# leonardsiegert/PULPo

Measured on AMD Instinct MI355X. Metric: volume-pairs/sec fwd+bwd, 160^3 fp32, higher is better.
Workload: dtype f32

## Files before the change

pulpo_amd/csrc/losses.hip:

```cpp
#include "common.h"

namespace {

inline int eblocks(long items, int cap = 4096) { return (int)std::max<long>(1, std::min<long>((items + 255) / 256, cap)); }

__device__ __forceinline__ float block_sum_256(float v, float* sh) {
    v = pulpo::wave_sum(v);
    if ((threadIdx.x & 63) == 0) sh[threadIdx.x >> 6] = v;
    __syncthreads();
    float t = 0.f;
    if (threadIdx.x == 0) t = sh[0] + sh[1] + sh[2] + sh[3];
    __syncthreads();
    return t;
}

__device__ __forceinline__ float ncc_cc(const float* s, float nwin) {
    const float uI = s[0] / nwin, uJ = s[1] / nwin;
    const float cross = s[4] - uJ * s[0] - uI * s[1] + uI * uJ * nwin;
    const float Iv = s[2] - 2.f * uI * s[0] + uI * uI * nwin;
    const float Jv = s[3] - 2.f * uJ * s[1] + uJ * uJ * nwin;
    return cross * cross / (Iv * Jv + 1e-8f);
}

__device__ __forceinline__ float mask_weight(const float* __restrict__ wa, const float* __restrict__ wb, long e) {
    return wb != nullptr ? wa[e] * wb[e] : wa[e];
}

template <bool MASKED>
__device__ __forceinline__ void store_block_partials(float local, float msum, float* sh, float* __restrict__ partial) {
    const float t = block_sum_256(local, sh);
    if constexpr (MASKED) {
        const float tm = block_sum_256(msum, sh);
        if (threadIdx.x == 0) {
            partial[2 * blockIdx.x] = t;
            partial[2 * blockIdx.x + 1] = tm;
        }
    } else {
        if (threadIdx.x == 0) partial[blockIdx.x] = t;
    }
}

template <int MODE>
__global__ __launch_bounds__(256) void box_x_kernel(const float* __restrict__ in0, const float* __restrict__ in1, float* __restrict__ out, long N,
                                                      long nrows, int W, int pad, int nch, int segs_per_row) {
    const int lane = threadIdx.x & 63;
    const int span = 64 - 2 * pad;
    const long nwork = nrows * segs_per_row;
    const long wave0 = (blockIdx.x * (long)blockDim.x + threadIdx.x) >> 6;
    const long nwave = ((long)gridDim.x * blockDim.x) >> 6;
    for (long wk = wave0; wk < nwork; wk += nwave) {
        const long row = wk / segs_per_row;
        const int seg = (int)(wk - row * segs_per_row);
        const int x = seg * span - pad + lane;
        const bool inb = x >= 0 && x < W;
        const long idx = row * W + x;
        const bool owner = lane >= pad && lane < 64 - pad && x < W;
        if constexpr (MODE == 0) {
            const float I = inb ? in0[idx] : 0.f, J = inb ? in1[idx] : 0.f;
            float v[5] = {I, J, I * I, J * J, I * J};
            float s[5] = {v[0], v[1], v[2], v[3], v[4]};
            for (int k = 1; k <= pad; ++k) {
#pragma unroll
                for (int c = 0; c < 5; ++c) s[c] += __shfl(v[c], lane - k, 64) + __shfl(v[c], lane + k, 64);
            }
            if (owner) {
#pragma unroll
                for (int c = 0; c < 5; ++c) out[c * N + idx] = s[c];
            }
        } else {
            for (int c = 0; c < nch; ++c) {
                const float v = inb ? in0[c * N + idx] : 0.f;
                float s = v;
                for (int k = 1; k <= pad; ++k) s += __shfl(v, lane - k, 64) + __shfl(v, lane + k, 64);
                if (owner) out[c * N + idx] = s;
            }
        }
    }
}

__global__ __launch_bounds__(256) void box_axis_kernel(const float* __restrict__ in, float* __restrict__ out, long N, int nch, int extent, long stride,
                                                         int pad) {
    for (long e = blockIdx.x * (long)blockDim.x + threadIdx.x; e < N; e += (long)gridDim.x * blockDim.x) {
        const int pos = (int)((e / stride) % extent);
        const int lo = max(-pad, -pos), hi = min(pad, extent - 1 - pos);
        for (int c = 0; c < nch; ++c) {
            const float* s = in + c * N + e;
            float acc = 0.f;
            for (int k = lo; k <= hi; ++k) acc += s[k * stride];
            out[c * N + e] = acc;
        }
    }
}

template <bool MASKED>
__global__ __launch_bounds__(256) void ncc_final_kernel(const float* __restrict__ in, float* __restrict__ S, long N, int extent, long stride, int pad,
                                                          float nwin, const float* __restrict__ wa, const float* __restrict__ wb, float* __restrict__ partial) {
    __shared__ float sh[4];
    float local = 0.f;
    [[maybe_unused]] float msum = 0.f;
    for (long e = blockIdx.x * (long)blockDim.x + threadIdx.x; e < N; e += (long)gridDim.x * blockDim.x) {
        const int pos = (int)((e / stride) % extent);
        const int lo = max(-pad, -pos), hi = min(pad, extent - 1 - pos);
        float s[5];
#pragma unroll
        for (int c = 0; c < 5; ++c) {
            const float* q = in + c * N + e;
            float acc = 0.f;
            for (int k = lo; k <= hi; ++k) acc += q[k * stride];
            s[c] = acc;
            S[c * N + e] = acc;
        }
        if constexpr (MASKED) {
            const float m = mask_weight(wa, wb, e);
            local += m * ncc_cc(s, nwin);
            msum += m;
        } else {
            local += ncc_cc(s, nwin);
        }
    }
    store_block_partials<MASKED>(local, msum, sh, partial);
}

template <int NCH, int PAD, int MODE, bool MASKED>
__global__ __launch_bounds__(256) void box_march_kernel(const float* __restrict__ in, float* __restrict__ out, long N, long nlines, int extent,
                                                          long stride, int seglen, int nseg, float nwin, float* __restrict__ partial,
                                                          const float* __restrict__ I, const float* __restrict__ J, const float* __restrict__ gscale,
                                                          float coef, const float* __restrict__ wa, const float* __restrict__ wb) {
    constexpr int WIN = 2 * PAD + 1;
    __shared__ float sh[4];
    const long nlg = (nlines + 255) / 256;
    const long nitem = nlg * nseg;
    float local = 0.f;
    [[maybe_unused]] float msum = 0.f;
    [[maybe_unused]] const float k0 = MODE == 2 ? coef * (gscale != nullptr ? gscale[0] : 1.f) : 0.f;
    for (long item = blockIdx.x; item < nitem; item += gridDim.x) {
        const long lg = item % nlg;
        const int seg = (int)(item / nlg);
        const long line = lg * 256 + threadIdx.x;
        if (line >= nlines) continue;
        const long outer = line / stride, inner = line - outer * stride;
        const long base = outer * extent * stride + inner;
        const int p0 = seg * seglen, p1 = min(extent, p0 + seglen);
        float ring[NCH][WIN];
#pragma unroll
        for (int j = 0; j < WIN - 1; ++j) {
            const int pos = p0 - PAD + j;
            const bool ok = pos >= 0 && pos < extent;
#pragma unroll
            for (int c = 0; c < NCH; ++c) ring[c][j] = ok ? in[c * N + base + pos * stride] : 0.f;
        }
        for (int t0 = p0; t0 < p1; t0 += WIN) {
#pragma unroll
            for (int u = 0; u < WIN; ++u) {
                const int p = t0 + u;
                if (p < p1) {
                    const int slot = (u + WIN - 1) % WIN;
                    const int pos = p + PAD;
                    const bool ok = pos < extent;
                    float sum[NCH];
#pragma unroll
                    for (int c = 0; c < NCH; ++c) {
                        ring[c][slot] = ok ? in[c * N + base + pos * stride] : 0.f;
                        float acc = 0.f;
#pragma unroll
                        for (int j = 0; j < WIN; ++j) acc += ring[c][(u + j) % WIN];
                        sum[c] = acc;
                    }
                    const long e = base + p * stride;
                    if constexpr (MODE == 0) {
#pragma unroll
                        for (int c = 0; c < NCH; ++c) out[c * N + e] = sum[c];
                    } else if constexpr (MODE == 1) {
#pragma unroll
                        for (int c = 0; c < NCH; ++c) out[c * N + e] = sum[c];
                        if constexpr (MASKED) {
                            const float m = mask_weight(wa, wb, e);
                            local += m * ncc_cc(sum, nwin);
                            msum += m;
                        } else {
                            local += ncc_cc(sum, nwin);
                        }
                    } else {
                        out[e] = k0 * (sum[0] + 2.f * J[e] * sum[1] + I[e] * sum[2]);
                    }
                }
            }
        }
    }
    if constexpr (MODE == 1) store_block_partials<MASKED>(local, msum, sh, partial);
}

static inline void march_segments(long nlines, int extent, int pad, int& seglen, int& nseg) {
    const long nlg = (nlines + 255) / 256;
    const long want = std::max<long>(1, (1024 + nlg - 1) / nlg);
    nseg = (int)std::max<long>(1, std::min<long>(want, extent / std::max(1, 2 * pad)));
    seglen = (extent + nseg - 1) / nseg;
    nseg = (extent + seglen - 1) / seglen;
}

template <int NCH, int MODE, bool MASKED = false>
static int launch_march(int pad, int grid, hipStream_t st, const float* in, float* out, long N, int extent, long stride, float nwin = 0.f,
                        float* partial = nullptr, const float* I = nullptr, const float* J = nullptr, const float* gscale = nullptr, float coef = 0.f,
                        const float* wa = nullptr, const float* wb = nullptr) {
    const long nlines = N / extent;
    int seglen, nseg;
    march_segments(nlines, extent, pad, seglen, nseg);
#define PULPO_MARCH(P) hipLaunchKernelGGL((box_march_kernel<NCH, P, MODE, MASKED>), dim3(grid), dim3(256), 0, st, in, out, N, nlines, extent, stride, seglen, nseg, nwin, partial, I, J, gscale, coef, wa, wb)
    switch (pad) {
        case 1: PULPO_MARCH(1); break;
        case 2: PULPO_MARCH(2); break;
        case 3: PULPO_MARCH(3); break;
        case 4: PULPO_MARCH(4); break;
        case 5: PULPO_MARCH(5); break;
        default: return -1;
    }
#undef PULPO_MARCH
    return pulpo::check_launch("ncc box march");
}

template <bool MASKED>
__global__ __launch_bounds__(256) void ncc_abc_kernel(const float* __restrict__ S, float* __restrict__ A, long N, float nwin,
                                                        const float* __restrict__ wa, const float* __restrict__ wb) {
    for (long e = blockIdx.x * (long)blockDim.x + threadIdx.x; e < N; e += (long)gridDim.x * blockDim.x) {
        const float SI = S[e], SJ = S[N + e], SII = S[2 * N + e], SJJ = S[3 * N + e], SIJ = S[4 * N + e];
        const float cross = SIJ - SI * SJ / nwin;
        const float Iv = SII - SI * SI / nwin;
        const float Jv = SJJ - SJ * SJ / nwin;
        const float Dn = Iv * Jv + 1e-8f;
        const float r = cross / Dn;
        float a = -2.f * r * SI / nwin + 2.f * r * r * Iv * SJ / nwin, b = -r * r * Iv, c = 2.f * r;
        if constexpr (MASKED) {
            const float m = mask_weight(wa, wb, e);
            a = m * a, b = m * b, c = m * c;
        }
        A[e] = a;
        A[N + e] = b;
        A[2 * N + e] = c;
    }
}

__global__ __launch_bounds__(256) void masked_finish_kernel(const float* __restrict__ partial, int nblk, double scale, int root, double count,
                                                              float* __restrict__ out) {
    __shared__ double red[2][256];
    double s = 0.0, m = 0.0;
    for (int r = threadIdx.x; r < nblk; r += 256) {
        s += (double)partial[2 * r];
        m += (double)partial[2 * r + 1];
    }
    red[0][threadIdx.x] = s;
    red[1][threadIdx.x] = m;
    __syncthreads();
    for (int half = 128; half > 0; half >>= 1) {
        if ((int)threadIdx.x < half) {
            red[0][threadIdx.x] += red[0][threadIdx.x + half];
            red[1][threadIdx.x] += red[1][threadIdx.x + half];
        }
        __syncthreads();
    }
    if (threadIdx.x == 0) {
        const double S0 = red[0][0], M = red[1][0];
        const bool live = M > 0.0;
        const double q = live ? scale * S0 / M : 0.0;
        double val = q, dval = live ? scale / M : 0.0;
        if (root) {
            val = q > 0.0 ? sqrt(q) : 0.0;
            dval = q > 0.0 ? dval / (2.0 * val) : 0.0;
        }
        out[0] = (float)val;
        out[1] = (float)dval;
        out[2] = (float)(M / count);
        out[3] = (float)M;
    }
}

__global__ __launch_bounds__(256) void ncc_bwd_final_kernel(const float* __restrict__ in, const float* __restrict__ I, const float* __restrict__ J,
                                                              const float* __restrict__ gscale, float coef, float* __restrict__ gJ, long N, int extent,
                                                              long stride, int pad) {
    const float k0 = coef * (gscale != nullptr ? gscale[0] : 1.f);
    for (long e = blockIdx.x * (long)blockDim.x + threadIdx.x; e < N; e += (long)gridDim.x * blockDim.x) {
        const int pos = (int)((e / stride) % extent);
        const int lo = max(-pad, -pos), hi = min(pad, extent - 1 - pos);
        float s[3];
#pragma unroll
        for (int c = 0; c < 3; ++c) {
            const float* q = in + c * N + e;
            float acc = 0.f;
            for (int k = lo; k <= hi; ++k) acc += q[k * stride];
            s[c] = acc;
        }
        gJ[e] = k0 * (s[0] + 2.f * J[e] * s[1] + I[e] * s[2]);
    }
}

__global__ __launch_bounds__(256) void kl_fwd_kernel(const float* __restrict__ mu, const float* __restrict__ sigma, const float* __restrict__ mu1,
                                                       const float* __restrict__ sigma1, long n, float* __restrict__ partial) {
    __shared__ float sh[4];
    float local = 0.f;
    const float eps = 1e-10f;
    for (long e = blockIdx.x * (long)blockDim.x + threadIdx.x; e < n; e += (long)gridDim.x * blockDim.x) {
        const float s0 = sigma[e] * sigma[e];
        const float s1 = sigma1 != nullptr ? sigma1[e] * sigma1[e] : 1.f;
        const float dm = (mu1 != nullptr ? mu1[e] : 0.f) - mu[e];
        local += (s0 + dm * dm) / (s1 + eps) + logf(s1 + eps) - logf(s0 + eps) - 1.f;
    }
    const float t = block_sum_256(local, sh);
    if (threadIdx.x == 0) partial[blockIdx.x] = t;
}

__global__ __launch_bounds__(256) void kl_bwd_kernel(const float* __restrict__ mu, const float* __restrict__ sigma, const float* __restrict__ mu1,
                                                       const float* __restrict__ sigma1, const float* __restrict__ gscale, float coef,
                                                       float* __restrict__ gmu, float* __restrict__ gsigma, long n) {
    const float k0 = coef * (gscale != nullptr ? gscale[0] : 1.f);
    const float eps = 1e-10f;
    for (long e = blockIdx.x * (long)blockDim.x + threadIdx.x; e < n; e += (long)gridDim.x * blockDim.x) {
        const float s = sigma[e], m = mu[e];
        const float s1 = sigma1 != nullptr ? sigma1[e] * sigma1[e] : 1.f;
        const float m1 = mu1 != nullptr ? mu1[e] : 0.f;
        gmu[e] = k0 * (m - m1) / (s1 + eps);
        gsigma[e] = k0 * (s / (s1 + eps) - s / (s * s + eps));
    }
}

__global__ __launch_bounds__(256) void l2reg_fwd_kernel(const float* __restrict__ df, long nplanes, int D, int H, int W, float* __restrict__ partial) {
    __shared__ float sh[4];
    float local = 0.f;
    const long V = (long)D * H * W, total = nplanes * V;
    for (long e = blockIdx.x * (long)blockDim.x + threadIdx.x; e < total; e += (long)gridDim.x * blockDim.x) {
        const long v = e % V;
        const int x = (int)(v % W), y = (int)((v / W) % H), z = (int)(v / ((long)W * H));
        if (x >= 1 && y >= 1 && (z >= 1 || D == 1)) {
            const float c = df[e];
            const float a = D == 1 ? 0.f : c - df[e - (long)H * W], b = c - df[e - W], d = c - df[e - 1];
            local += a * a + b * b + d * d;
        }
    }
    const float t = block_sum_256(local, sh);
    if (threadIdx.x == 0) partial[blockIdx.x] = t;
}

__global__ __launch_bounds__(256) void l2reg_fwd_vec_kernel(const float* __restrict__ df, long nplanes, int D, int H, int W, float* __restrict__ partial) {
    __shared__ float sh[4];
    float local = 0.f;
    const int W4 = W >> 2;
    const long items = nplanes * D * H * W4;
    for (long it = blockIdx.x * (long)blockDim.x + threadIdx.x; it < items; it += (long)gridDim.x * blockDim.x) {
        const int x4 = (int)(it % W4);
        const long row = it / W4;
        const int y = (int)(row % H);
        const int z = (int)((row / H) % D);
        if (y >= 1 && (z >= 1 || D == 1)) {
            const long e = row * W + 4 * x4;
            const float4 c = *reinterpret_cast<const float4*>(df + e);
            const float4 u = *reinterpret_cast<const float4*>(df + e - W);
            float4 bk = c;
            if (D != 1) bk = *reinterpret_cast<const float4*>(df + e - (long)H * W);
            const float cc[4] = {c.x, c.y, c.z, c.w}, uu[4] = {u.x, u.y, u.z, u.w}, bb[4] = {bk.x, bk.y, bk.z, bk.w};
            float left = x4 > 0 ? df[e - 1] : 0.f;
#pragma unroll
            for (int k = 0; k < 4; ++k) {
                if (4 * x4 + k >= 1) {
                    const float a = cc[k] - bb[k], b = cc[k] - uu[k], d = cc[k] - left;
                    local += a * a + b * b + d * d;
                }
                left = cc[k];
            }
        }
    }
    const float t = block_sum_256(local, sh);
    if (threadIdx.x == 0) partial[blockIdx.x] = t;
}

__global__ __launch_bounds__(256) void l2reg_bwd_vec_kernel(const float* __restrict__ df, const float* __restrict__ gscale, float coef,
                                                              float* __restrict__ gdf, long nplanes, int D, int H, int W) {
    const float k0 = 2.f * coef * (gscale != nullptr ? gscale[0] : 1.f);
    const int W4 = W >> 2;
    const long items = nplanes * D * H * W4;
    const long sz = (long)H * W;
    const bool flat = D == 1;
    const float4 zero = make_float4(0.f, 0.f, 0.f, 0.f);
    for (long it = blockIdx.x * (long)blockDim.x + threadIdx.x; it < items; it += (long)gridDim.x * blockDim.x) {
        const int x4 = (int)(it % W4);
        const long row = it / W4;
        const int y = (int)(row % H);
        const int z = (int)((row / H) % D);
        const long e = row * W + 4 * x4;
        const float4 c = *reinterpret_cast<const float4*>(df + e);
        const float4 zm = (z >= 1) ? *reinterpret_cast<const float4*>(df + e - sz) : zero;
        const float4 zp = (z + 1 < D) ? *reinterpret_cast<const float4*>(df + e + sz) : zero;
        const float4 ym = (y >= 1) ? *reinterpret_cast<const float4*>(df + e - W) : zero;
        const float4 yp = (y + 1 < H) ? *reinterpret_cast<const float4*>(df + e + W) : zero;
        const float xm = x4 > 0 ? df[e - 1] : 0.f, xp = x4 + 1 < W4 ? df[e + 4] : 0.f;
        const float cc[4] = {c.x, c.y, c.z, c.w}, a0[4] = {zm.x, zm.y, zm.z, zm.w}, a1[4] = {zp.x, zp.y, zp.z, zp.w};
        const float b0[4] = {ym.x, ym.y, ym.z, ym.w}, b1[4] = {yp.x, yp.y, yp.z, yp.w};
        float o[4];
#pragma unroll
        for (int k = 0; k < 4; ++k) {
            const int x = 4 * x4 + k;
            const float cv = cc[k];
            const float lft = k > 0 ? cc[k - 1] : xm, rgt = k < 3 ? cc[k + 1] : xp;
            float g = 0.f;
            if (x >= 1 && y >= 1 && (z >= 1 || flat)) g += (flat ? 0.f : cv - a0[k]) + (cv - b0[k]) + (cv - lft);
            if (z + 1 < D && y >= 1 && x >= 1) g -= a1[k] - cv;
            if (y + 1 < H && (z >= 1 || flat) && x >= 1) g -= b1[k] - cv;
            if (x + 1 < W && (z >= 1 || flat) && y >= 1) g -= rgt - cv;
            o[k] = k0 * g;
        }
        *reinterpret_cast<float4*>(gdf + e) = make_float4(o[0], o[1], o[2], o[3]);
    }
}

__global__ __launch_bounds__(256) void l2reg_bwd_kernel(const float* __restrict__ df, const float* __restrict__ gscale, float coef,
                                                          float* __restrict__ gdf, long nplanes, int D, int H, int W) {
    const float k0 = 2.f * coef * (gscale != nullptr ? gscale[0] : 1.f);
    const long V = (long)D * H * W, total = nplanes * V;
    const long sz = (long)H * W, sy = W;
    for (long e = blockIdx.x * (long)blockDim.x + threadIdx.x; e < total; e += (long)gridDim.x * blockDim.x) {
        const long v = e % V;
        const int x = (int)(v % W), y = (int)((v / W) % H), z = (int)(v / sz);
        const float c = df[e];
        float g = 0.f;
        const bool flat = D == 1;
        if (x >= 1 && y >= 1 && (z >= 1 || flat)) g += (flat ? 0.f : c - df[e - sz]) + (c - df[e - sy]) + (c - df[e - 1]);
        if (z + 1 < D && y >= 1 && x >= 1) g -= df[e + sz] - c;
        if (y + 1 < H && (z >= 1 || flat) && x >= 1) g -= df[e + sy] - c;
        if (x + 1 < W && (z >= 1 || flat) && y >= 1) g -= df[e + 1] - c;
        gdf[e] = k0 * g;
    }
}

}

PULPO_API int pulpo_loss_blocks(int64_t n) { return eblocks(n, 1024); }

static inline float ncc_window_count(int win, int D) { return D == 1 ? (float)(win * win) : (float)(win * win * win); }

#define PULPO_NCC_REQUIRE(name, pointers)                                                  \
    PULPO_REQUIRE((pointers) && B > 0 && D > 0 && H > 0 && W > 0, name ": bad arguments"); \
    PULPO_REQUIRE(win >= 1 && (win & 1) && win <= 31, name ": window must be odd and <= 31")

static int ncc_forward(const float* I, const float* J, const float* wa, const float* wb, float* S, float* T, float* partial, int B, int D, int H, int W,
                       int win, hipStream_t st) {
    const long N = (long)B * D * H * W;
    const int pad = win / 2, span = 64 - 2 * pad, segs = pulpo::cdiv(W, span);
    const long nrows = (long)B * D * H;
    const float nwin = ncc_window_count(win, D);
    float* T1 = T;
    float* T2 = T + 5 * N;
    hipLaunchKernelGGL(box_x_kernel<0>, dim3(eblocks(nrows * segs * 64)), dim3(256), 0, st, I, J, T1, N, nrows, W, pad, 5, segs);
    int rc = pulpo::check_launch("ncc box_x");
    if (rc) return rc;
    const bool march = pad >= 1 && pad <= 5;
    if (march && H > 1) rc = launch_march<5, 0>(pad, eblocks(N, 1024), st, T1, T2, N, H, (long)W);
    else {
        hipLaunchKernelGGL(box_axis_kernel, dim3(eblocks(N)), dim3(256), 0, st, T1, T2, N, 5, H, (long)W, pad);
        rc = pulpo::check_launch("ncc box_y");
    }
    if (rc) return rc;
    const int grid = pulpo_loss_blocks(N);
    const long stride = (long)H * W;
    if (march && wa) return launch_march<5, 1, true>(pad, grid, st, T2, S, N, D, stride, nwin, partial, nullptr, nullptr, nullptr, 0.f, wa, wb);
    if (march) return launch_march<5, 1>(pad, grid, st, T2, S, N, D, stride, nwin, partial);
    if (wa) hipLaunchKernelGGL(ncc_final_kernel<true>, dim3(grid), dim3(256), 0, st, T2, S, N, D, stride, pad, nwin, wa, wb, partial);
    else hipLaunchKernelGGL(ncc_final_kernel<false>, dim3(grid), dim3(256), 0, st, T2, S, N, D, stride, pad, nwin, wa, wb, partial);
    return pulpo::check_launch("ncc final");
}

static int ncc_backward(const float* I, const float* J, const float* S, const float* wa, const float* wb, float* T, const float* gscale, float coef,
                        float* gJ, int B, int D, int H, int W, int win, hipStream_t st) {
    const long N = (long)B * D * H * W;
    const int pad = win / 2, span = 64 - 2 * pad, segs = pulpo::cdiv(W, span);
    const long nrows = (long)B * D * H;
    float* T1 = T;
    float* T2 = T + 3 * N;
    if (wa) hipLaunchKernelGGL(ncc_abc_kernel<true>, dim3(eblocks(N)), dim3(256), 0, st, S, T1, N, ncc_window_count(win, D), wa, wb);
    else hipLaunchKernelGGL(ncc_abc_kernel<false>, dim3(eblocks(N)), dim3(256), 0, st, S, T1, N, ncc_window_count(win, D), wa, wb);
    int rc = pulpo::check_launch("ncc abc");
    if (rc) return rc;
    hipLaunchKernelGGL(box_x_kernel<1>, dim3(eblocks(nrows * segs * 64)), dim3(256), 0, st, T1, nullptr, T2, N, nrows, W, pad, 3, segs);
    rc = pulpo::check_launch("ncc bwd box_x");
    if (rc) return rc;
    const bool march = pad >= 1 && pad <= 5;
    if (march && H > 1) rc = launch_march<3, 0>(pad, eblocks(N, 1024), st, T2, T1, N, H, (long)W);
    else {
        hipLaunchKernelGGL(box_axis_kernel, dim3(eblocks(N)), dim3(256), 0, st, T2, T1, N, 3, H, (long)W, pad);
        rc = pulpo::check_launch("ncc bwd box_y");
    }
    if (rc) return rc;
    if (march) return launch_march<3, 2>(pad, eblocks(N, 1024), st, T1, gJ, N, D, (long)H * W, 0.f, nullptr, I, J, gscale, coef);
    hipLaunchKernelGGL(ncc_bwd_final_kernel, dim3(eblocks(N)), dim3(256), 0, st, T1, I, J, gscale, coef, gJ, N, D, (long)H * W, pad);
    return pulpo::check_launch("ncc bwd final");
}

PULPO_API int pulpo_ncc_fwd(const float* I, const float* J, float* S, float* T, float* partial, int B, int D, int H, int W, int win, void* stream) {
    PULPO_NCC_REQUIRE("ncc_fwd", I && J && S && T && partial);
    return ncc_forward(I, J, nullptr, nullptr, S, T, partial, B, D, H, W, win, (hipStream_t)stream);
}

PULPO_API int pulpo_ncc_bwd(const float* I, const float* J, const float* S, float* T, const float* gscale, float coef, float* gJ, int B, int D, int H,
                            int W, int win, void* stream) {
    PULPO_NCC_REQUIRE("ncc_bwd", I && J && S && T && gJ);
    return ncc_backward(I, J, S, nullptr, nullptr, T, gscale, coef, gJ, B, D, H, W, win, (hipStream_t)stream);
}

PULPO_API int pulpo_ncc_masked_fwd(const float* I, const float* J, const float* wa, const float* wb, float* S, float* T, float* partial, int B, int D,
                                   int H, int W, int win, void* stream) {
    PULPO_NCC_REQUIRE("ncc_masked_fwd", I && J && wa && S && T && partial);
    return ncc_forward(I, J, wa, wb, S, T, partial, B, D, H, W, win, (hipStream_t)stream);
}

PULPO_API int pulpo_ncc_masked_bwd(const float* I, const float* J, const float* S, const float* wa, const float* wb, float* T, const float* gscale,
                                   float coef, float* gJ, int B, int D, int H, int W, int win, void* stream) {
    PULPO_NCC_REQUIRE("ncc_masked_bwd", I && J && S && wa && T && gJ);
    return ncc_backward(I, J, S, wa, wb, T, gscale, coef, gJ, B, D, H, W, win, (hipStream_t)stream);
}
#undef PULPO_NCC_REQUIRE

PULPO_API int pulpo_masked_finish(const float* partial, int nblk, double scale, int root, double count, float* out, void* stream) {
    PULPO_REQUIRE(partial && out && nblk > 0 && count > 0, "masked_finish: bad arguments");
    hipLaunchKernelGGL(masked_finish_kernel, dim3(1), dim3(256), 0, (hipStream_t)stream, partial, nblk, scale, root, count, out);
    return pulpo::check_launch("masked_finish");
}

PULPO_API int pulpo_kl_fwd(const float* mu, const float* sigma, const float* mu1, const float* sigma1, int64_t n, float* partial, void* stream) {
    PULPO_REQUIRE(mu && sigma && partial && n > 0, "kl_fwd: bad arguments");
    hipLaunchKernelGGL(kl_fwd_kernel, dim3(pulpo_loss_blocks(n)), dim3(256), 0, (hipStream_t)stream, mu, sigma, mu1, sigma1, (long)n, partial);
    return pulpo::check_launch("kl_fwd");
}

PULPO_API int pulpo_kl_bwd(const float* mu, const float* sigma, const float* mu1, const float* sigma1, const float* gscale, float coef, float* gmu,
                           float* gsigma, int64_t n, void* stream) {
    PULPO_REQUIRE(mu && sigma && gmu && gsigma && n > 0, "kl_bwd: bad arguments");
    hipLaunchKernelGGL(kl_bwd_kernel, dim3(eblocks(n)), dim3(256), 0, (hipStream_t)stream, mu, sigma, mu1, sigma1, gscale, coef, gmu, gsigma, (long)n);
    return pulpo::check_launch("kl_bwd");
}

PULPO_API int pulpo_l2reg_fwd(const float* df, int64_t nplanes, int D, int H, int W, float* partial, void* stream) {
    PULPO_REQUIRE(df && partial && nplanes > 0 && D >= 1 && H > 1 && W > 1, "l2reg_fwd: bad arguments");
    if (W % 4 == 0 && (((uintptr_t)df) & 15) == 0)
        hipLaunchKernelGGL(l2reg_fwd_vec_kernel, dim3(pulpo_loss_blocks(nplanes * D * H * W)), dim3(256), 0, (hipStream_t)stream, df, (long)nplanes, D, H, W, partial);
    else
        hipLaunchKernelGGL(l2reg_fwd_kernel, dim3(pulpo_loss_blocks(nplanes * D * H * W)), dim3(256), 0, (hipStream_t)stream, df, (long)nplanes, D, H, W, partial);
    return pulpo::check_launch("l2reg_fwd");
}

PULPO_API int pulpo_l2reg_bwd(const float* df, const float* gscale, float coef, float* gdf, int64_t nplanes, int D, int H, int W, void* stream) {
    PULPO_REQUIRE(df && gdf && nplanes > 0 && D >= 1 && H > 1 && W > 1, "l2reg_bwd: bad arguments");
    if (W % 4 == 0 && ((((uintptr_t)df) | ((uintptr_t)gdf)) & 15) == 0)
        hipLaunchKernelGGL(l2reg_bwd_vec_kernel, dim3(eblocks(nplanes * D * H * (W / 4))), dim3(256), 0, (hipStream_t)stream, df, gscale, coef, gdf, (long)nplanes, D, H, W);
    else
        hipLaunchKernelGGL(l2reg_bwd_kernel, dim3(eblocks(nplanes * D * H * W)), dim3(256), 0, (hipStream_t)stream, df, gscale, coef, gdf, (long)nplanes, D, H, W);
    return pulpo::check_launch("l2reg_bwd");
}

namespace {
__global__ void weighted_sum_fwd_kernel(const float* __restrict__ t, const float* __restrict__ w, int n, float scale, int scaled, float* __restrict__ levels,
                                        float* __restrict__ total) {
    if (threadIdx.x == 0 && blockIdx.x == 0) {
        float s = 0.f;
        for (int i = 0; i < n; ++i) {
            const float v = __fmul_rn(w[i], t[i]);
            s = __fadd_rn(s, v);
            levels[i] = scaled ? __fmul_rn(v, scale) : v;
        }
        total[0] = scaled ? __fmul_rn(s, scale) : s;
    }
}
__global__ void weighted_sum_bwd_kernel(const float* __restrict__ gtotal, const float* __restrict__ glevels, const float* __restrict__ w, int n, float scale,
                                        float* __restrict__ gt) {
    const int i = threadIdx.x;
    if (blockIdx.x == 0 && i < n) {
        const float a = gtotal ? __fmul_rn(gtotal[0], scale) : 0.f;
        const float b = glevels ? __fmul_rn(glevels[i], scale) : 0.f;
        gt[i] = __fmul_rn(__fadd_rn(a, b), w[i]);
    }
}
}

PULPO_API int pulpo_weighted_sum_fwd(const float* terms, const float* weights, int n, float scale, int scaled, float* levels, float* total, void* stream) {
    PULPO_REQUIRE(terms && weights && levels && total && n > 0 && n <= 64, "weighted_sum_fwd: bad arguments");
    hipLaunchKernelGGL(weighted_sum_fwd_kernel, dim3(1), dim3(64), 0, (hipStream_t)stream, terms, weights, n, scale, scaled, levels, total);
    return pulpo::check_launch("weighted_sum_fwd");
}

PULPO_API int pulpo_weighted_sum_bwd(const float* gtotal, const float* glevels, const float* weights, int n, float scale, float* gterms, void* stream) {
    PULPO_REQUIRE((gtotal || glevels) && weights && gterms && n > 0 && n <= 64, "weighted_sum_bwd: bad arguments");
    hipLaunchKernelGGL(weighted_sum_bwd_kernel, dim3(1), dim3(64), 0, (hipStream_t)stream, gtotal, glevels, weights, n, scale, gterms);
    return pulpo::check_launch("weighted_sum_bwd");
}
```

Measured before the change: 39.69.

## Fuse NCC box filters into tiled single-pass forward and backward kernels

Replaces the multi-kernel separable box-filter chain (x pass, y march, z march, plus a separate abc kernel in backward) with one tiled kernel per direction. Each block stages an XY halo tile in shared memory, does the x and y sums there, and keeps a z ring buffer in registers while marching through depth segments, with next-slice global loads prefetched. The backward kernel computes the a/b/c coefficients on the fly and uses a reciprocal-with-correction divide. This removes the intermediate T buffers and several full-volume global round trips, at the cost of halo recomputation, more register pressure, and barriers on every slice.

```diff
diff --git a/pulpo_amd/csrc/losses.hip b/pulpo_amd/csrc/losses.hip
--- a/pulpo_amd/csrc/losses.hip
+++ b/pulpo_amd/csrc/losses.hip
@@ -1,3 +1,5 @@
+#include <stdlib.h>
+
 #include "common.h"
 
 namespace {
@@ -218,17 +220,32 @@
     return pulpo::check_launch("ncc box march");
 }
 
+template <bool RCP>
+__device__ __forceinline__ float ncc_over(float x, float nwin, float rn) {
+    if constexpr (RCP) {
+        const float q = x * rn;
+        return __builtin_fmaf(__builtin_fmaf(-q, nwin, x), rn, q);
+    } else {
+        return x / nwin;
+    }
+}
+
+template <bool RCP = false>
+__device__ __forceinline__ void ncc_abc(float SI, float SJ, float SII, float SJJ, float SIJ, float nwin, float rn, float& a, float& b, float& c) {
+    const float cross = SIJ - ncc_over<RCP>(SI * SJ, nwin, rn);
+    const float Iv = SII - ncc_over<RCP>(SI * SI, nwin, rn);
+    const float Jv = SJJ - ncc_over<RCP>(SJ * SJ, nwin, rn);
+    const float Dn = Iv * Jv + 1e-8f;
+    const float r = cross / Dn;
+    a = ncc_over<RCP>(-2.f * r * SI, nwin, rn) + ncc_over<RCP>(2.f * r * r * Iv * SJ, nwin, rn), b = -r * r * Iv, c = 2.f * r;
+}
+
 template <bool MASKED>
 __global__ __launch_bounds__(256) void ncc_abc_kernel(const float* __restrict__ S, float* __restrict__ A, long N, float nwin,
                                                         const float* __restrict__ wa, const float* __restrict__ wb) {
     for (long e = blockIdx.x * (long)blockDim.x + threadIdx.x; e < N; e += (long)gridDim.x * blockDim.x) {
-        const float SI = S[e], SJ = S[N + e], SII = S[2 * N + e], SJJ = S[3 * N + e], SIJ = S[4 * N + e];
-        const float cross = SIJ - SI * SJ / nwin;
-        const float Iv = SII - SI * SI / nwin;
-        const float Jv = SJJ - SJ * SJ / nwin;
-        const float Dn = Iv * Jv + 1e-8f;
-        const float r = cross / Dn;
-        float a = -2.f * r * SI / nwin + 2.f * r * r * Iv * SJ / nwin, b = -r * r * Iv, c = 2.f * r;
+        float a, b, c;
+        ncc_abc(S[e], S[N + e], S[2 * N + e], S[3 * N + e], S[4 * N + e], nwin, 0.f, a, b, c);
         if constexpr (MASKED) {
             const float m = mask_weight(wa, wb, e);
             a = m * a, b = m * b, c = m * c;
@@ -237,6 +254,273 @@
         A[N + e] = b;
         A[2 * N + e] = c;
     }
+}
+
+constexpr int NCC_TX = 32, NCC_FWD_TY = 8, NCC_BWD_TY = 16;
+
+struct NccTile {
+    int b, y0, x0, p0, p1;
+};
+
+template <int TY>
+__device__ __forceinline__ NccTile ncc_tile(int item, int nitem, int ntx, int nty, int seglen, int nseg, int D) {
+    int r = pulpo::xcd_remap(item, nitem);
+    NccTile t;
+    t.x0 = (r % ntx) * NCC_TX, r /= ntx;
+    t.y0 = (r % nty) * TY, r /= nty;
+    t.p0 = (r % nseg) * seglen, t.b = r / nseg;
+    t.p1 = min(D, t.p0 + seglen);
+    return t;
+}
+
+template <int PAD, int TY, int NLD>
+__device__ __forceinline__ void ncc_halo_slots(const NccTile& t, int H, int W, int* off, bool* ok) {
+    constexpr int HX = NCC_TX + 2 * PAD, NH = HX * (TY + 2 * PAD);
+#pragma unroll
+    for (int k = 0; k < NLD; ++k) {
+        const int h = threadIdx.x + NCC_TX * TY * k;
+        const int gy = t.y0 - PAD + h / HX, gx = t.x0 - PAD + h % HX;
+        ok[k] = h < NH && gy >= 0 && gy < H && gx >= 0 && gx < W;
+        off[k] = ok[k] ? gy * W + gx : 0;
+    }
+}
+
+template <int PAD>
+__device__ __forceinline__ float ncc_ysum(const float (*xs)[NCC_TX], int ty, int tx) {
+    float acc = 0.f;
+#pragma unroll
+    for (int j = 0; j < 2 * PAD + 1; ++j) acc += xs[ty + j][tx];
+    return acc;
+}
+
+template <int PAD, bool MASKED>
+__global__ __launch_bounds__(NCC_TX * NCC_FWD_TY) void ncc_fwd_tiled_kernel(const float* __restrict__ I, const float* __restrict__ J, float* __restrict__ S, long N,
+                                                              int D, int H, int W, int ntx, int nty, int seglen, int nseg, int nitem, float nwin,
+                                                              const float* __restrict__ wa, const float* __restrict__ wb,
+                                                              float* __restrict__ partial) {
+    constexpr int TY = NCC_FWD_TY, NT = NCC_TX * TY, WIN = 2 * PAD + 1, HX = NCC_TX + 2 * PAD, HY = TY + 2 * PAD, NH = HX * HY, NLD = (NH + NT - 1) / NT;
+    __shared__ float sI[NH], sJ[NH];
+    __shared__ float xs[5][HY][NCC_TX];
+    __shared__ float sh[4];
+    const int tx = threadIdx.x % NCC_TX, ty = threadIdx.x / NCC_TX;
+    const int plane = H * W;
+    float local = 0.f;
+    [[maybe_unused]] float msum = 0.f;
+    for (int item = blockIdx.x; item < nitem; item += gridDim.x) {
+        const NccTile t = ncc_tile<TY>(item, nitem, ntx, nty, seglen, nseg, D);
+        const long vol0 = (long)t.b * D * plane;
+        const float* Ib = I + vol0;
+        const float* Jb = J + vol0;
+        int off[NLD];
+        bool ok[NLD];
+        ncc_halo_slots<PAD, TY, NLD>(t, H, W, off, ok);
+        const int y = t.y0 + ty, x = t.x0 + tx;
+        const bool owner = y < H && x < W;
+        const int own = y * W + x;
+        float ring[5][WIN];
+#pragma unroll
+        for (int c = 0; c < 5; ++c)
+#pragma unroll
+            for (int j = 0; j < WIN; ++j) ring[c][j] = 0.f;
+        float nI[NLD], nJ[NLD];
+        const int q0 = t.p0 - PAD, q1 = t.p1 + PAD;
+#pragma unroll
+        for (int k = 0; k < NLD; ++k) {
+            const bool ld = ok[k] && q0 >= 0;
+            nI[k] = ld ? Ib[q0 * plane + off[k]] : 0.f;
+            nJ[k] = ld ? Jb[q0 * plane + off[k]] : 0.f;
+        }
+#pragma unroll 1
+        for (int q = q0; q < q1; ++q) {
+            const bool live = q >= 0 && q < D;
+            float v[5] = {0.f, 0.f, 0.f, 0.f, 0.f};
+            if (live) {
+#pragma unroll
+                for (int k = 0; k < NLD; ++k) {
+                    const int h = threadIdx.x + NT * k;
+                    if (h < NH) sI[h] = nI[k], sJ[h] = nJ[k];
+                }
+                __syncthreads();
+            }
+            {
+                const int qn = q + 1;
+                const bool nlive = qn < q1 && qn >= 0 && qn < D;
+#pragma unroll
+                for (int k = 0; k < NLD; ++k) {
+                    const bool ld = ok[k] && nlive;
+                    nI[k] = ld ? Ib[qn * plane + off[k]] : 0.f;
+                    nJ[k] = ld ? Jb[qn * plane + off[k]] : 0.f;
+                }
+            }
+            if (live) {
+                for (int r = ty; r < HY; r += TY) {
+#pragma clang fp contract(off)
+                    const float* ri = sI + r * HX + tx + PAD;
+                    const float* rj = sJ + r * HX + tx + PAD;
+                    const float ic = ri[0], jc = rj[0];
+                    float s0 = ic, s1 = jc, s2 = ic * ic, s3 = jc * jc, s4 = ic * jc;
+#pragma unroll
+                    for (int k = 1; k <= PAD; ++k) {
+                        const float il = ri[-k], ir = ri[k], jl = rj[-k], jr = rj[k];
+                        s0 += il + ir;
+                        s1 += jl + jr;
+                        s2 += il * il + ir * ir;
+                        s3 += jl * jl + jr * jr;
+                        s4 += il * jl + ir * jr;
+                    }
+                    xs[0][r][tx] = s0, xs[1][r][tx] = s1, xs[2][r][tx] = s2, xs[3][r][tx] = s3, xs[4][r][tx] = s4;
+                }
+                __syncthreads();
+#pragma unroll
+                for (int c = 0; c < 5; ++c) v[c] = ncc_ysum<PAD>(xs[c], ty, tx);
+            }
+            float sum[5];
+#pragma unroll
+            for (int c = 0; c < 5; ++c) {
+#pragma unroll
+                for (int j = 0; j < WIN - 1; ++j) ring[c][j] = ring[c][j + 1];
+                ring[c][WIN - 1] = v[c];
+                float acc = 0.f;
+#pragma unroll
+                for (int j = 0; j < WIN; ++j) acc += ring[c][j];
+                sum[c] = acc;
+            }
+            const int p = q - PAD;
+            if (p >= t.p0 && owner) {
+                const long e = vol0 + p * plane + own;
+#pragma unroll
+                for (int c = 0; c < 5; ++c) S[c * N + e] = sum[c];
+                if constexpr (MASKED) {
+                    const float m = mask_weight(wa, wb, e);
+                    local += m * ncc_cc(sum, nwin);
+                    msum += m;
+                } else {
+                    local += ncc_cc(sum, nwin);
+                }
+            }
+        }
+    }
+    store_block_partials<MASKED>(local, msum, sh, partial);
+}
+
+template <int PAD, bool MASKED>
+__global__ __launch_bounds__(NCC_TX * NCC_BWD_TY) void ncc_bwd_tiled_kernel(const float* __restrict__ I, const float* __restrict__ J, const float* __restrict__ S,
+                                                              float* __restrict__ gJ, long N, int D, int H, int W, int ntx, int nty, int seglen,
+                                                              int nseg, int nitem, float nwin, const float* __restrict__ gscale, float coef,
+                                                              const float* __restrict__ wa, const float* __restrict__ wb) {
+    constexpr int TY = NCC_BWD_TY, NT = NCC_TX * TY, WIN = 2 * PAD + 1, HX = NCC_TX + 2 * PAD, HY = TY + 2 * PAD, NH = HX * HY, NLD = (NH + NT - 1) / NT;
+    __shared__ float sA[3][NH];
+    __shared__ float xs[3][HY][NCC_TX];
+    const int tx = threadIdx.x % NCC_TX, ty = threadIdx.x / NCC_TX;
+    const int plane = H * W;
+    const float k0 = coef * (gscale != nullptr ? gscale[0] : 1.f);
+    const float rn = 1.f / nwin;
+    for (int item = blockIdx.x; item < nitem; item += gridDim.x) {
+        const NccTile t = ncc_tile<TY>(item, nitem, ntx, nty, seglen, nseg, D);
+        const long vol0 = (long)t.b * D * plane;
+        const float* Sb = S + vol0;
+        int off[NLD];
+        bool ok[NLD];
+        ncc_halo_slots<PAD, TY, NLD>(t, H, W, off, ok);
+        const int y = t.y0 + ty, x = t.x0 + tx;
+        const bool owner = y < H && x < W;
+        const int own = y * W + x;
+        float ring[3][WIN];
+#pragma unroll
+        for (int c = 0; c < 3; ++c)
+#pragma unroll
+            for (int j = 0; j < WIN; ++j) ring[c][j] = 0.f;
+        float nS[5][NLD];
+        [[maybe_unused]] float nM[NLD];
+        const int q0 = t.p0 - PAD, q1 = t.p1 + PAD;
+#pragma unroll
+        for (int k = 0; k < NLD; ++k) {
+            const bool ld = ok[k] && q0 >= 0;
+#pragma unroll
+            for (int c = 0; c < 5; ++c) nS[c][k] = ld ? Sb[c * N + q0 * plane + off[k]] : 0.f;
+            if constexpr (MASKED) nM[k] = ld ? mask_weight(wa, wb, vol0 + q0 * plane + off[k]) : 0.f;
+        }
+#pragma unroll 1
+        for (int q = q0; q < q1; ++q) {
+            const bool live = q >= 0 && q < D;
+            const int p = q - PAD;
+            const bool emit = p >= t.p0 && owner;
+            const long e = vol0 + (emit ? p * plane + own : 0);
+            const float Ie = emit ? I[e] : 0.f, Je = emit ? J[e] : 0.f;
+            float v[3] = {0.f, 0.f, 0.f};
+            if (live) {
+#pragma unroll
+                for (int k = 0; k < NLD; ++k) {
+                    const int h = threadIdx.x + NT * k;
+                    float a = 0.f, b = 0.f, c = 0.f;
+                    if (ok[k]) {
+                        ncc_abc<true>(nS[0][k], nS[1][k], nS[2][k], nS[3][k], nS[4][k], nwin, rn, a, b, c);
+                        if constexpr (MASKED) a = nM[k] * a, b = nM[k] * b, c = nM[k] * c;
+                    }
+                    if (h < NH) sA[0][h] = a, sA[1][h] = b, sA[2][h] = c;
+                }
+                __syncthreads();
+            }
+            {
+                const int qn = q + 1;
+                const bool nlive = qn < q1 && qn >= 0 && qn < D;
+#pragma unroll
+                for (int k = 0; k < NLD; ++k) {
+                    const bool ld = ok[k] && nlive;
+#pragma unroll
+                    for (int c = 0; c < 5; ++c) nS[c][k] = ld ? Sb[c * N + qn * plane + off[k]] : 0.f;
+                    if constexpr (MASKED) nM[k] = ld ? mask_weight(wa, wb, vol0 + qn * plane + off[k]) : 0.f;
+                }
+            }
+            if (live) {
+                for (int r = ty; r < HY; r += TY) {
+#pragma unroll
+                    for (int c = 0; c < 3; ++c) {
+                        const float* ra = sA[c] + r * HX + tx + PAD;
+                        float s = ra[0];
+#pragma unroll
+                        for (int k = 1; k <= PAD; ++k) s += ra[-k] + ra[k];
+                        xs[c][r][tx] = s;
+                    }
+                }
+                __syncthreads();
+#pragma unroll
+                for (int c = 0; c < 3; ++c) v[c] = ncc_ysum<PAD>(xs[c], ty, tx);
+            }
+            float sum[3];
+#pragma unroll
+            for (int c = 0; c < 3; ++c) {
+#pragma unroll
+                for (int j = 0; j < WIN - 1; ++j) ring[c][j] = ring[c][j + 1];
+                ring[c][WIN - 1] = v[c];
+                float acc = 0.f;
+#pragma unroll
+                for (int j = 0; j < WIN; ++j) acc += ring[c][j];
+                sum[c] = acc;
+            }
+            if (emit) gJ[e] = k0 * (sum[0] + 2.f * Je * sum[1] + Ie * sum[2]);
+        }
+    }
+}
+
+static inline bool ncc_tile_geometry(int B, int D, int H, int W, int ty, int slots, int& ntx, int& nty, int& seglen, int& nseg, int& nitem) {
+    if ((long)D * H * W >= (1L << 31)) return false;
+    ntx = pulpo::cdiv(W, NCC_TX), nty = pulpo::cdiv(H, ty);
+    const long npatch = (long)B * ntx * nty;
+    nseg = (int)std::max<long>(1, std::min<long>(slots / npatch, D));
+    seglen = (D + nseg - 1) / nseg;
+    nseg = (D + seglen - 1) / seglen;
+    if (npatch * nseg >= (1L << 31)) return false;
+    nitem = (int)(npatch * nseg);
+    return true;
+}
+
+static bool ncc_tiled_enabled() {
+    static const bool on = [] {
+        const char* v = getenv("PULPO_NCC_TILED");
+        return !(v != nullptr && v[0] == '0' && v[1] == '\0');
+    }();
+    return on;
 }
 
 __global__ __launch_bounds__(256) void masked_finish_kernel(const float* __restrict__ partial, int nblk, double scale, int root, double count,
@@ -444,6 +728,24 @@
     const int pad = win / 2, span = 64 - 2 * pad, segs = pulpo::cdiv(W, span);
     const long nrows = (long)B * D * H;
     const float nwin = ncc_window_count(win, D);
+    int ntx, nty, seglen, nseg, nitem;
+    const int grid = pulpo_loss_blocks(N);
+    if (ncc_tiled_enabled() && D > 1 && pad >= 1 && pad <= 5 && ncc_tile_geometry(B, D, H, W, NCC_FWD_TY, grid, ntx, nty, seglen, nseg, nitem)) {
+#define PULPO_TILED(P)                                                                                                                            \
+    if (wa) hipLaunchKernelGGL((ncc_fwd_tiled_kernel<P, true>), dim3(grid), dim3(NCC_TX * NCC_FWD_TY), 0, st, I, J, S, N, D, H, W, ntx, nty, seglen, nseg, nitem, \
+                               nwin, wa, wb, partial);                                                                                            \
+    else hipLaunchKernelGGL((ncc_fwd_tiled_kernel<P, false>), dim3(grid), dim3(NCC_TX * NCC_FWD_TY), 0, st, I, J, S, N, D, H, W, ntx, nty, seglen, nseg, nitem,   \
+                            nwin, wa, wb, partial)
+        switch (pad) {
+            case 1: PULPO_TILED(1); break;
+            case 2: PULPO_TILED(2); break;
+            case 3: PULPO_TILED(3); break;
+            case 4: PULPO_TILED(4); break;
+            default: PULPO_TILED(5); break;
+        }
+#undef PULPO_TILED
+        return pulpo::check_launch("ncc fwd tiled");
+    }
     float* T1 = T;
     float* T2 = T + 5 * N;
     hipLaunchKernelGGL(box_x_kernel<0>, dim3(eblocks(nrows * segs * 64)), dim3(256), 0, st, I, J, T1, N, nrows, W, pad, 5, segs);
@@ -456,7 +758,6 @@
         rc = pulpo::check_launch("ncc box_y");
     }
     if (rc) return rc;
-    const int grid = pulpo_loss_blocks(N);
     const long stride = (long)H * W;
     if (march && wa) return launch_march<5, 1, true>(pad, grid, st, T2, S, N, D, stride, nwin, partial, nullptr, nullptr, nullptr, 0.f, wa, wb);
     if (march) return launch_march<5, 1>(pad, grid, st, T2, S, N, D, stride, nwin, partial);
@@ -470,6 +771,25 @@
     const long N = (long)B * D * H * W;
     const int pad = win / 2, span = 64 - 2 * pad, segs = pulpo::cdiv(W, span);
     const long nrows = (long)B * D * H;
+    int ntx, nty, seglen, nseg, nitem;
+    if (ncc_tiled_enabled() && D > 1 && pad >= 1 && pad <= 5 && ncc_tile_geometry(B, D, H, W, NCC_BWD_TY, 512, ntx, nty, seglen, nseg, nitem)) {
+        const int grid = std::min(nitem, 2048);
+        const float nwin = ncc_window_count(win, D);
+#define PULPO_TILED(P)                                                                                                                             \
+    if (wa) hipLaunchKernelGGL((ncc_bwd_tiled_kernel<P, true>), dim3(grid), dim3(NCC_TX * NCC_BWD_TY), 0, st, I, J, S, gJ, N, D, H, W, ntx, nty, seglen, nseg,     \
+                               nitem, nwin, gscale, coef, wa, wb);                                                                                 \
+    else hipLaunchKernelGGL((ncc_bwd_tiled_kernel<P, false>), dim3(grid), dim3(NCC_TX * NCC_BWD_TY), 0, st, I, J, S, gJ, N, D, H, W, ntx, nty, seglen, nseg,       \
+                            nitem, nwin, gscale, coef, wa, wb)
+        switch (pad) {
+            case 1: PULPO_TILED(1); break;
+            case 2: PULPO_TILED(2); break;
+            case 3: PULPO_TILED(3); break;
+            case 4: PULPO_TILED(4); break;
+            default: PULPO_TILED(5); break;
+        }
+#undef PULPO_TILED
+        return pulpo::check_launch("ncc bwd tiled");
+    }
     float* T1 = T;
     float* T2 = T + 3 * N;
     if (wa) hipLaunchKernelGGL(ncc_abc_kernel<true>, dim3(eblocks(N)), dim3(256), 0, st, S, T1, N, ncc_window_count(win, D), wa, wb);
```

Measured after the change: 39.97 (median of 6 runs). Within noise of the previous version (+0.7%).
